# buttomnutstoast/Multigrid-Neural-Architectures

Hardware: NVIDIA B200
Metric: R-MG-34 train images/sec (higher is better)
Workload: dtype bf16

## Files before the change

### include/mgconv.h

```cpp
#ifndef MGCONV_H
#define MGCONV_H

#include <stdint.h>
#include <stddef.h>

#ifdef __cplusplus
extern "C" {
#endif

enum {
  MG_MAX_SEG = 6,
  MG_MAX_SRC = 8
};

typedef struct mg_ctx mg_ctx;

typedef enum {
  MG_OK = 0,
  MG_ERR_INVALID_ARG = 1,
  MG_ERR_SHAPE = 2,
  MG_ERR_CUDA = 3,
  MG_ERR_NCCL = 4,
  MG_ERR_UNSUPPORTED = 5
} mg_status;

typedef enum { MG_F32 = 0, MG_BF16 = 1 } mg_dtype;

typedef enum {
  MG_SEG_SAME = 0,
  MG_SEG_POOL = 1,
  MG_SEG_UP = 2
} mg_seg_mode;

typedef enum { MG_IMPL_AUTO = 0, MG_IMPL_SIMT = 1, MG_IMPL_TCGEN05 = 2 } mg_impl;

typedef struct { int64_t hi, lo; } mg_sum;

typedef struct {
  void* data;
  const float* scale;
  const float* shift;
  int32_t relu;
  int32_t N, H, W, C, Cp;
} mg_grid;

typedef struct {
  int32_t n_seg;
  mg_grid seg[MG_MAX_SEG];
  int32_t seg_mode[MG_MAX_SEG];
  int32_t ksize, stride, pad;
  int32_t Cout;
  int32_t H, W;
  int32_t algo_fwd, algo_bwd_data;
} mg_conv_desc;
enum { MG_ALGO_AUTO = 0, MG_ALGO_TILE128 = 1,
       MG_ALGO_TILE256 = 2,
       MG_ALGO_RESIDENT = 3,
       MG_ALGO_TILE128_DEEP = 4,
       MG_ALGO_TILE256_DEEP = 5,
       MG_ALGO_TILE128_MID = 6,
       MG_ALGO_PAIR128 = 7,
       MG_ALGO_PAIR256 = 8,
       MG_ALGO_RESIDENT_PAIR = 9 };

typedef struct {
  mg_grid g;
  int32_t c_offset;
  int32_t mode;
  const void* aux;
} mg_grad_src;

int mg_ctx_create(int device, void* cuda_stream, int dtype, mg_ctx** out);
int mg_ctx_destroy(mg_ctx* ctx);
int mg_ctx_set_stream(mg_ctx* ctx, void* cuda_stream);
int mg_ctx_set_impl(mg_ctx* ctx, int impl);
int mg_ctx_lane(mg_ctx* ctx, int lane);
int mg_ctx_event_record(mg_ctx* ctx, int ev);
int mg_ctx_event_wait(mg_ctx* ctx, int ev);
int mg_ctx_sync(mg_ctx* ctx);
enum { MG_TUNE_HALO_SUBTILES = 0,
       MG_TUNE_PERSISTENT = 1,
       MG_TUNE_STEM_FUSED_STATS = 2  };
int mg_ctx_set_tuning(mg_ctx* ctx, int knob, int value);
const char* mg_last_error(mg_ctx* ctx);
int mg_version(void);
int mg_ctx_launch_count(mg_ctx* ctx, int64_t* out);
int mg_ctx_tc_launch_count(mg_ctx* ctx, int64_t* out);
int mg_ctx_profile(mg_ctx* ctx, int on);
int mg_ctx_profile_read(mg_ctx* ctx, double* conv_ms, int64_t* conv_calls);

int mg_import_nchw(mg_ctx* ctx, const float* src, mg_grid* dst);
int mg_export_nchw(mg_ctx* ctx, const mg_grid* src, float* dst);

int mg_crop_flip_normalize(mg_ctx* ctx, const float* src, int32_t N, int32_t C, int32_t H, int32_t W, float* dst, int32_t oH, int32_t oW,
                           const int32_t* y0, const int32_t* x0, const int32_t* flip, const float* mean, const float* stdv);

size_t mg_conv_packed_bytes(const mg_conv_desc* d, int transposed);
int mg_conv_pack_weights(mg_ctx* ctx, const mg_conv_desc* d, const float* w, void* wpack, int transposed);
int mg_conv_pack_weights_batched(mg_ctx* ctx, int32_t n, const mg_conv_desc* const* descs, const float* const* w,
                                 void* const* wpack, const int32_t* transposed);

int mg_conv_forward(mg_ctx* ctx, const mg_conv_desc* d, const float* w, const void* wpack,
                    const float* bias, mg_grid* y, mg_sum* bn_sums);

int mg_bn_finalize(mg_ctx* ctx, const mg_sum* bn_sums, int64_t count, int32_t C, int32_t Cp,
                   const float* gamma, const float* beta, float* running_mean, float* running_var,
                   float eps, float momentum, int training,
                   float* scale, float* shift, float* save_mean, float* save_invstd);

int mg_residual_forward(mg_ctx* ctx, const mg_grid* z, const mg_grid* s, int relu, mg_grid* out, mg_grid* pooled);

typedef struct {
  const mg_sum* sums;
  int64_t count;
  const float* gamma;
  const float* beta;
// ... 89 lines not shown
```

### multigrid-neural-architectures_b200/csrc/umma_conv.cu

```cuda
#include "common.cuh"
#include "conv_view.cuh"
#include "umma_common.cuh"
#include "tma.cuh"
#include <algorithm>
#include <vector>

namespace {

constexpr int BM = 128;
constexpr int KV_PER_STAGE = 8;
constexpr int A_STAGE_BYTES = BM * 128;
constexpr int N_PRODUCERS = 128;
constexpr int MMA_WARP = 4, B_WARP = 5;
constexpr int N_THREADS = 192;
constexpr int MAX_STAGES = 8;

struct UParams {
  USeg seg[MG_MAX_SEG];
  int n_seg;
  int k, stride, pad;
  int H, W;
  int Ho, Wo;
  int64_t M;
  int Nimg;
// ... 267 lines not shown
    }
  }
  __syncthreads();
  if (warp == MMA_WARP) {
    tc_fence_after();
    asm volatile("tcgen05.dealloc.cta_group::1.sync.aligned.b32 %0, %1;" ::"r"(tmem_base), "r"(p.tmem_cols) : "memory");
  }
}



__device__ __forceinline__ float warp_reduce_scatter16(float (&v)[16], int lane) {
#pragma unroll
  for (int o = 8; o >= 1; o >>= 1) {
    const bool hi = (lane & o) != 0;
#pragma unroll
    for (int i = 0; i < o; ++i) {
      const float send = hi ? v[i] : v[i + o];
      const float keep = hi ? v[i + o] : v[i];
      v[i] = keep + __shfl_xor_sync(0xffffffffu, send, o);
    }
  }
  return v[0] + __shfl_xor_sync(0xffffffffu, v[0], 16);
}

constexpr int MAX_CHUNKS = 32;
struct HChunk { int seg, c0, nch, tps, ksteps, stage0; };

struct HParams {
  CUtensorMap tmap[MG_MAX_SEG];
  int seg_up[MG_MAX_SEG];
  HChunk chunk[MAX_CHUNKS];
  int n_seg, n_chunks, n_stages, any_up;
  int img_box;
  int H, W, Wp, Hp, Nimg;
  int64_t T;
  int HL;
  int nr_max;
  int halo_bytes;
  int n_abuf;
  int n_tile;
  const uint8_t* wpack;
  const float* bias;
  int c_bias;
  __nv_bfloat16* y;
  int y_pitch, c_valid;
  int stages, tmem_cols;
  mg_sum* stats;
  int c_stats;
  int m_tiles;
  CUtensorMap tmap_w;
  int tile_rows;
  int epi_stage;
};

__device__ __forceinline__ void zero_pad_column(uint8_t* a_smem, int nbuf, int halo_bytes, int nr_max, int Wp, int tid, int nthreads, int org = 0) {
  for (int i = tid; i < nbuf * nr_max * 8; i += nthreads) {
    const int q = i & 7, row = (i >> 3) % nr_max, buf = (i >> 3) / nr_max;
    *reinterpret_cast<uint4*>(a_smem + (size_t)buf * halo_bytes + (size_t)(org + row * Wp + Wp - 1) * 128 + q * 16) = make_uint4(0, 0, 0, 0);
  }
  fence_proxy_async();
}

__device__ __forceinline__ void zero_halo_margins(uint8_t* a_smem, int nbuf, int halo_bytes, int HL, int Wp, int tid, int nthreads) {
  const int m = Wp + 1;
  for (int i = tid; i < nbuf * 2 * m * 8; i += nthreads) {
    const int q = i & 7, sl = (i >> 3) % (2 * m), buf = (i >> 3) / (2 * m);
    const int slot = sl < m ? sl : HL - 2 * m + sl;
    *reinterpret_cast<uint4*>(a_smem + (size_t)buf * halo_bytes + (size_t)slot * 128 + q * 16) = make_uint4(0, 0, 0, 0);
  }
  fence_proxy_async();
}

__device__ __forceinline__ bool slot_pixel(const HParams& p, int64_t t, uint32_t* pix) {
  if (t >= p.T) return false;
  const uint32_t tu = (uint32_t)t, spi = (uint32_t)(p.Hp * p.Wp);
  const uint32_t n = tu / spi, rem = tu - n * spi;
  const uint32_t yy = rem / (uint32_t)p.Wp, xs = rem - yy * (uint32_t)p.Wp;
  if ((int)yy >= p.H || (int)xs >= p.W) return false;
  *pix = (n * p.H + yy) * p.W + xs;
  return true;
}

template <int MT>
__global__ void __launch_bounds__(32 * (4 * MT + 3), MT == 1 ? 4 : 2) umma_conv_halo_kernel(const __grid_constant__ HParams p) {
  constexpr int EPI_WARPS = 4 * MT, A_WARP = EPI_WARPS, B_WARP = EPI_WARPS + 1, M_WARP = EPI_WARPS + 2, NT = 32 * (EPI_WARPS + 3);
  extern __shared__ __align__(1024) uint8_t smem_raw[];
  uint8_t* smem = (uint8_t*)(((uintptr_t)smem_raw + 1023) & ~(uintptr_t)1023);
  __shared__ uint64_t full_bar[MAX_STAGES], empty_bar[MAX_STAGES], a_full[2], a_empty[2], tmem_full_bar;
  __shared__ uint32_t tmem_base_s;
  __shared__ float s_bias[256];

  pdl_launch();
  const int tid = threadIdx.x, warp = tid >> 5, lane = tid & 31;
  const int S = p.stages;
  const int b_stage_bytes = p.n_tile * 128;
  uint8_t* a_smem = smem;
  uint8_t* b_smem = smem + (size_t)p.n_abuf * p.halo_bytes;
  const int t0 = (int)blockIdx.x * (BM * MT);
  const int ntile = blockIdx.y;
  const int hs = t0 - p.Wp - 1;
  const int r0 = floordiv(hs, p.Wp);
  const int nr = (hs + p.HL - 1) / p.Wp - r0 + 1;
  const int off = p.img_box ? 0 : hs - r0 * p.Wp;

  if (tid == 0) {
// ... 735 lines not shown
          tma_load_rows_pair(&p.tmap[ch.seg], up, dst, &a_full[buf], ch.c0, r0, nr, p.W, p.Hp, lane);
        }
      }
    }
  } else if (warp == P_B_WARP) {
    if (lane == 0) {
      if (rank == 0) mbar_arrive_expect_tx(&b_full, (uint32_t)(2 * p.n_stages * b_half_bytes));
      for (int q = 0; q < p.n_stages; ++q)
        tma_load_2d_pair(smem_u32(b_smem + (size_t)q * b_half_bytes), &p.tmap_w, &b_full, 0, q * p.n_tile + (int)rank * (p.n_tile >> 1));
    }
  } else if (rank == 0) {
    const bool leader = elect_one();
    const uint32_t idesc = (1u << 4) | (1u << 7) | (1u << 10) | ((uint32_t)(p.n_tile >> 3) << 17) | ((uint32_t)(256 >> 4) << 24);
    const uint32_t b_base = smem_u32(b_smem);
    Ring ra(NA);
    mbar_wait_cluster(&b_full, 0);
    for (int it = 0; it < n_my; ++it) {
      const int acc = it & 1;
      if (it >= 2) { mbar_wait_cluster(&tmem_empty[acc], ((it >> 1) - 1) & 1); tc_fence_after(); }
      const uint32_t d_tmem = tmem_base + (uint32_t)(acc * p.n_tile);
      for (int c = 0; c < p.n_chunks; ++c, ra.next()) {
        const int buf = ra.idx;
        const HChunk ch = p.chunk[c];
        mbar_wait_cluster(&a_full[buf], ra.phase);
        tc_fence_after();
        const uint32_t a_base = smem_u32(a_smem + (size_t)buf * p.halo_bytes);
        const int tps = ch.tps, ksteps = ch.ksteps;
        const uint32_t sub_lo = 8u / (uint32_t)tps;
        if (leader) {
          int sub = 0, st = ch.stage0;
          for (int tap = 0; tap < 9; ++tap) {
            const uint32_t a_lo = desc_lo_k_sw128(a_base + (uint32_t)((tap / 3) * p.Wp + (tap % 3)) * 128u);
            const uint32_t b_lo = desc_lo_k_sw128(b_base + (uint32_t)(st * b_half_bytes)) + (uint32_t)sub * sub_lo;
#pragma unroll
            for (int q = 0; q < 4; ++q)
              if (q < ksteps) tc_mma_bf16_lohi_pair(d_tmem, a_lo + (uint32_t)(q * 2), b_lo + (uint32_t)(q * 2), DESC_HI_SW128, idesc, (uint32_t)((c | tap | q) != 0));
            if (++sub == tps) { sub = 0; ++st; }
          }
          tc_commit_pair(&a_empty[buf]);
        }
      }
      if (leader) tc_commit_pair(&tmem_full[acc]);
    }
  }
  __syncthreads();
  cluster_sync_all();
  if (warp == P_MMA_WARP) {
    tc_fence_after();
    asm volatile("tcgen05.dealloc.cta_group::2.sync.aligned.b32 %0, %1;" ::"r"(tmem_base), "r"(p.tmem_cols) : "memory");
  }
}


constexpr int ST_PC = 11, ST_PR = 37;
constexpr int ST_ROW = ST_PC * 16;
constexpr int ST_PLANE = 6592;
constexpr int ST_SLOT = 13312;
constexpr int ST_MAX_RING = 6;
constexpr int ST_RAW_COLS = 21;
constexpr int ST_RAW = 12544;
constexpr int ST_THREADS = 480;

struct StemParams {
  CUtensorMap tmap;
  CUtensorMap tmap_y;
  int tma_out;
  int H, W, Ho, Wo, Nimg;
  int tiles_x, tiles_y, n_tiles_total;
  int n_tile;
  int ring;
  const uint8_t* wpack;
  const float* bias; int c_bias;
  __nv_bfloat16* y; int y_pitch, c_valid;
  mg_sum* stats; int c_stats;
  int tmem_cols;
};

__device__ __forceinline__ uint64_t smem_desc_k_none(uint32_t saddr, uint32_t lbo_bytes, uint32_t sbo_bytes) {
  return (uint64_t)((saddr >> 4) & 0x3FFF) | ((uint64_t)((lbo_bytes >> 4) & 0x3FFF) << 16) | ((uint64_t)((sbo_bytes >> 4) & 0x3FFF) << 32) | (1ull << 46);
}

__global__ void __launch_bounds__(ST_THREADS, 1) umma_stem_kernel(const __grid_constant__ StemParams p) {
  pdl_launch();
  extern __shared__ __align__(1024) uint8_t smem_raw[];
  uint8_t* smem = (uint8_t*)(((uintptr_t)smem_raw + 1023) & ~(uintptr_t)1023);
  __shared__ uint64_t b_full, r_full[ST_MAX_RING], r_empty[ST_MAX_RING], a_full[ST_MAX_RING], a_empty[ST_MAX_RING], tmem_full[2], tmem_empty[2];
  __shared__ uint32_t tmem_base_s;

  const int tid = threadIdx.x, warp = tid >> 5, lane = tid & 31;
  const int NA = p.ring;
  const int b_stage_bytes = p.n_tile * 128;
  uint8_t* b_smem = smem;
  uint8_t* a_smem = smem + 7 * b_stage_bytes;
  uint8_t* r_smem = a_smem + (size_t)NA * ST_SLOT;
  uint8_t* o_smem = r_smem + (size_t)NA * ST_RAW;
  long long* s_part = reinterpret_cast<long long*>(o_smem + (p.tma_out ? 2 * 16384 : 0));
  float* s_bias = reinterpret_cast<float*>(s_part + 32 * p.n_tile);
  const int n_my = (p.n_tiles_total - (int)blockIdx.x + (int)gridDim.x - 1) / (int)gridDim.x;

  for (int c = tid; c < 32 * p.n_tile; c += ST_THREADS) s_part[c] = 0;
  if (tid == 0) {
    mbar_init(&b_full, 1);
    for (int s = 0; s < NA; ++s) { mbar_init(&a_full[s], 128); mbar_init(&a_empty[s], 1); mbar_init(&r_full[s], 1); mbar_init(&r_empty[s], 128); }
    for (int s = 0; s < 2; ++s) { mbar_init(&tmem_full[s], 1); mbar_init(&tmem_empty[s], 128); }
    asm volatile("fence.mbarrier_init.release.cluster;" ::: "memory");
  }
// ... 373 lines not shown
  if (!attr_set) {
    MG_CUDA(ctx, cudaFuncSetAttribute(umma_conv_kernel<true>, cudaFuncAttributeMaxDynamicSharedMemorySize, 227 * 1024 - 8 * 1024));
    MG_CUDA(ctx, cudaFuncSetAttribute(umma_conv_kernel<false>, cudaFuncAttributeMaxDynamicSharedMemorySize, 227 * 1024 - 8 * 1024));
    attr_set = true;
  }
  dim3 grid((unsigned)mg_cdiv(p.M, BM), (unsigned)n_tiles);
  bool fast = p.stride == 1 && (p.k == 1 || p.k == 3) && p.pad == p.k / 2 && p.Ho == p.H && p.Wo == p.W && p.M < (int64_t)1 << 31;
  for (int s = 0; s < p.n_seg; ++s) {
    if (p.seg[s].shift) fast = fast && p.seg[s].Hs == p.H / 2 && p.seg[s].Ws == p.W / 2 && p.H % 2 == 0 && p.W % 2 == 0;
    else fast = fast && p.seg[s].Hs == p.H && p.seg[s].Ws == p.W;
  }
  if (fast) umma_conv_kernel<true><<<grid, N_THREADS, smem, ctx->stream>>>(p);
  else umma_conv_kernel<false><<<grid, N_THREADS, smem, ctx->stream>>>(p);
  MG_CHECK_LAUNCH(ctx);
  ctx->tc_launches++;
  return MG_OK;
}

constexpr int SMEM_MAX = 232448 - 4096;

static void halo_geometry(HParams& p, int slots) {
  p.HL = slots + 2 * p.Wp + 2;
  p.nr_max = (p.HL - 1 + p.Wp - 1) / p.Wp + 1;
  p.halo_bytes = mg_round_up((p.img_box ? p.HL : p.nr_max * p.Wp) * 128, 1024);
}

static bool img_box_ok(const HParams& p, int slots) {
  static int on = -1;
  if (on < 0) { const char* e = getenv("MGCONV_IMG_BOX"); on = e ? atoi(e) : 1; }
  const int spi = p.Hp * p.Wp;
  return on && !p.any_up && slots % spi == 0 && slots / spi <= 256;
}

static int halo_tensor_maps(mg_ctx* ctx, HParams& p, const mg_grid* segs, int slots) {
  p.img_box = img_box_ok(p, slots) ? 1 : 0;
  for (int s = 0; s < p.n_seg; ++s) {
    const mg_grid& g = segs[s];
    int rc = p.img_box ? mg_tensor_map(ctx, g.data, p.Nimg, g.H, g.W, g.Cp, 4, slots / (p.Hp * p.Wp), &p.tmap[s])
                       : mg_tensor_map(ctx, g.data, p.Nimg, g.H, g.W, g.Cp, p.seg_up[s] ? 1 : 0, p.seg_up[s] ? 2 * g.W : p.Wp, &p.tmap[s]);
    if (rc) return rc;
  }
  return MG_OK;
}

static int epilogue_staging(const HParams& p, int MT, int smem_usable) {
  static int on = -1;
  if (on < 0) { const char* e = getenv("MGCONV_EPI_STAGE"); on = e ? atoi(e) : 1; }
  if (!on) return 0;
  const int off = p.stats ? MT * 4 * 2 * 256 * 4 : 0;
  const int need = off + MT * BM * (p.n_tile * 2 + 16);
  return need <= smem_usable ? off + 1 : 0;
}

static int launch_halo(mg_ctx* ctx, HParams& p, const Geometry& g, int algo, const mg_grid* segs) {
  const int b_stage = p.n_tile * 128;
  static int budget_env = -1, mt_env = -1;
  if (budget_env < 0) { const char* e = getenv("MGCONV_HALO_SMEM_KB"); budget_env = e ? atoi(e) : 0; }
  if (mt_env < 0) { const char* e = getenv("MGCONV_MT"); mt_env = e ? atoi(e) : 0; }
  int MT;
  {
    const int64_t ctas2 = mg_cdiv(p.T, 2 * BM) * g.n_tiles;
    const int want = (algo == MG_ALGO_TILE128 || algo == MG_ALGO_TILE128_DEEP || algo == MG_ALGO_TILE128_MID) ? 1
                     : ((algo == MG_ALGO_TILE256 || algo == MG_ALGO_TILE256_DEEP) ? 2 : (ctx->tune_mt ? ctx->tune_mt : mt_env));
    const bool heur2 = g.n_chunks >= 3 && ctas2 * 10 >= (int64_t)ctx->num_sms * 8;
    MT = (want == 1 || want == 2) ? want : (heur2 ? 2 : 1);
  }
  const bool pair = algo == MG_ALGO_PAIR128 || algo == MG_ALGO_PAIR256;
  if (pair) MT = algo == MG_ALGO_PAIR256 ? 2 : 1;
  { int rc = halo_tensor_maps(ctx, p, segs, BM * MT); if (rc) return rc; }
  halo_geometry(p, BM * MT);
  int cols = 32;
  while (cols < MT * p.n_tile) cols <<= 1;
  p.tmem_cols = cols;
  if (pair) {
    if (!p.img_box) p.halo_bytes = mg_round_up((p.nr_max * p.Wp + p.Wp) * 128, 1024);
    const int half = b_stage / 2;
    const int ctas = std::max(1, std::min(512 / cols, 2));
    int budget = (budget_env > 0 ? budget_env : (ctas == 1 ? 200 : 108)) * 1024;
    p.n_abuf = (g.n_chunks > 1 && 2 * p.halo_bytes + 2 * half <= budget) ? 2 : 1;
    int S = (budget - p.n_abuf * p.halo_bytes) / half;
    S = std::max(2, std::min(S, std::min(MAX_STAGES, p.n_stages)));
    p.stages = S;
    const int smem = p.n_abuf * p.halo_bytes + S * half + 1024;
    MG_REQUIRE(ctx, smem <= SMEM_MAX, MG_ERR_UNSUPPORTED, "pair halo conv: %d bytes of shared memory", smem);
    p.epi_stage = epilogue_staging(p, MT, smem - 1024);
    int rc = mg_tensor_map(ctx, p.wpack, g.n_tiles * p.n_stages * p.n_tile, 0, 0, 0, 5, p.n_tile / 2, &p.tmap_w);
    if (rc) return rc;
    static bool pair_attr_set = false;
    if (!pair_attr_set) {
      MG_CUDA(ctx, cudaFuncSetAttribute(umma_conv_halo_pair_kernel<1>, cudaFuncAttributeMaxDynamicSharedMemorySize, SMEM_MAX));
      MG_CUDA(ctx, cudaFuncSetAttribute(umma_conv_halo_pair_kernel<2>, cudaFuncAttributeMaxDynamicSharedMemorySize, SMEM_MAX));
      pair_attr_set = true;
    }
    dim3 grid((unsigned)mg_round_up((int)mg_cdiv(p.T, BM * MT), 2), (unsigned)g.n_tiles);
    if (MT == 2) MG_CUDA(ctx, mg_launch_pdl(umma_conv_halo_pair_kernel<2>, grid, dim3(32 * 11), (size_t)smem, ctx->stream, p));
    else MG_CUDA(ctx, mg_launch_pdl(umma_conv_halo_pair_kernel<1>, grid, dim3(32 * 7), (size_t)smem, ctx->stream, p));
    MG_CHECK_LAUNCH(ctx);
    ctx->tc_launches++;
    return MG_OK;
  }
  int budget_kb;
  if (MT == 1) {
    budget_kb = p.n_tile >= 192 ? 108 : 56;
  } else {
    const int ctas = std::max(1, std::min(512 / cols, 2));
    budget_kb = ctas == 1 ? 200 : 108;
  }
  if (algo == MG_ALGO_TILE128_MID) budget_kb = 72;
  if ((algo == MG_ALGO_AUTO || algo == MG_ALGO_RESIDENT) && mg_cdiv(p.T, BM * MT) * g.n_tiles <= ctx->num_sms) budget_kb = 200;
  if (algo == MG_ALGO_TILE128_DEEP) budget_kb = 108;
  if (algo == MG_ALGO_TILE256_DEEP) budget_kb = 200;
  if (budget_env > 0) budget_kb = budget_env;
  const int min_ring = 2;
  p.n_abuf = (g.n_chunks > 1 && 2 * p.halo_bytes + min_ring * b_stage <= budget_kb * 1024) ? 2 : 1;
  int S = (budget_kb * 1024 - p.n_abuf * p.halo_bytes) / b_stage;
  S = std::max(2, std::min(S, std::min(MAX_STAGES, p.n_stages)));
  p.stages = S;
  static bool attr_set = false;
  if (!attr_set) {
    MG_CUDA(ctx, cudaFuncSetAttribute(umma_conv_halo_kernel<1>, cudaFuncAttributeMaxDynamicSharedMemorySize, SMEM_MAX));
    MG_CUDA(ctx, cudaFuncSetAttribute(umma_conv_halo_kernel<2>, cudaFuncAttributeMaxDynamicSharedMemorySize, SMEM_MAX));
    attr_set = true;
  }
  const int smem = p.n_abuf * p.halo_bytes + S * b_stage + 1024;
  MG_REQUIRE(ctx, smem <= SMEM_MAX, MG_ERR_UNSUPPORTED, "halo conv: %d bytes of shared memory", smem);
  p.epi_stage = epilogue_staging(p, MT, smem - 1024);
  dim3 grid((unsigned)mg_cdiv(p.T, BM * MT), (unsigned)g.n_tiles);
  if (MT == 2) MG_CUDA(ctx, mg_launch_pdl(umma_conv_halo_kernel<2>, grid, dim3(32 * 11), (size_t)smem, ctx->stream, p));
  else MG_CUDA(ctx, mg_launch_pdl(umma_conv_halo_kernel<1>, grid, dim3(32 * 7), (size_t)smem, ctx->stream, p));
  MG_CHECK_LAUNCH(ctx);
  ctx->tc_launches++;
  return MG_OK;
}

struct PersistPlan { int n_abuf, smem, tmem_cols, grid, tile_rows, halo_bytes, pair; };
static int persist_tile_rows(const mg_conv_desc* d, int Nimg, bool any_up) {
  const int Wp = d->W + 1, Hp = d->H + 1;
  if (Wp > BM) return 0;
  if (!any_up && BM % (Hp * Wp) == 0) return 0;
  const int R = BM / Wp;
  if (R < 1 || R * Wp * 100 < BM * 85) return 0;
  (void)Nimg;
  return R;
}
static bool persist_plan(const mg_ctx* ctx, const mg_conv_desc* d, const Geometry& g, int Nimg, int algo, bool stats, PersistPlan* pl) {
  static int on = -1, min_tiles_per_sm = -1;
  if (on < 0) { const char* e = getenv("MGCONV_PERSIST"); on = e ? atoi(e) : 1; }
  if (min_tiles_per_sm < 0) { const char* e = getenv("MGCONV_PERSIST_MIN_TILES"); min_tiles_per_sm = e ? atoi(e) : 4; }
  if (algo == MG_ALGO_TILE128 || algo == MG_ALGO_TILE256 || algo == MG_ALGO_TILE128_DEEP || algo == MG_ALGO_TILE256_DEEP ||
      algo == MG_ALGO_TILE128_MID || algo == MG_ALGO_PAIR128 || algo == MG_ALGO_PAIR256) return false;
  const bool pair = algo == MG_ALGO_RESIDENT_PAIR;
  const bool forced = algo == MG_ALGO_RESIDENT || pair || ctx->tune_persist == 1;
  if (!forced && (ctx->tune_persist == 2 || !on)) return false;
  if (!g.halo || g.n_tiles != 1) return false;
  HParams hp;
  hp.Wp = d->W + 1; hp.img_box = 0;
  halo_geometry(hp, BM);
  bool any_up = false;
  for (int s = 0; s < d->n_seg; ++s) any_up = any_up || d->seg_mode[s] == MG_SEG_UP;
  static int aligned_single = -1;
  if (aligned_single < 0) { const char* e = getenv("MGCONV_PERSIST_ALIGNED"); aligned_single = e ? atoi(e) : 0; }
  const int R = ((pair || aligned_single) && !stats) ? persist_tile_rows(d, Nimg, any_up && g.n_chunks > 0) : 0;
  if (R) hp.halo_bytes = mg_round_up(((R + 2) * hp.Wp + 2) * 128, 1024);
  const int64_t m_tiles = R ? mg_cdiv((int64_t)Nimg * (d->H + 1), R) : mg_cdiv((int64_t)Nimg * (d->H + 1) * hp.Wp, BM);
  if (!forced && m_tiles < (int64_t)min_tiles_per_sm * ctx->num_sms) return false;
  if (pair && !R && !(!any_up && BM % ((d->H + 1) * hp.Wp) == 0)) return false;
  const int b_bytes = g.n_stages * g.n_tile * (pair ? 64 : 128);
  const int tail = g.n_tile * (4 + 256);
  const int room = SMEM_MAX - 1024 - b_bytes - tail;
  int n_abuf = room / hp.halo_bytes;
  if (n_abuf < 2) return false;
  n_abuf = std::min(n_abuf, std::min(P_MAX_ABUF, 2 * g.n_chunks + 1));
  int cols = 32;
  while (cols < 2 * g.n_tile) cols <<= 1;
  if (cols > 512) return false;
  pl->n_abuf = n_abuf; pl->smem = n_abuf * hp.halo_bytes + b_bytes + tail + 1024; pl->tmem_cols = cols;
  pl->grid = (int)std::min<int64_t>(m_tiles, ctx->num_sms);
  if (pair) pl->grid = 2 * (int)std::min<int64_t>((m_tiles + 1) / 2, ctx->num_sms / 2);
  pl->tile_rows = R; pl->halo_bytes = hp.halo_bytes; pl->pair = pair ? 1 : 0;
  return true;
}

static int launch_halo_persistent(mg_ctx* ctx, HParams& p, const PersistPlan& pl, const mg_grid* segs) {
  { int rc = halo_tensor_maps(ctx, p, segs, BM); if (rc) return rc; }
  halo_geometry(p, BM);
  p.m_tiles = (int)mg_cdiv(p.T, BM);
  p.tile_rows = p.img_box ? 0 : pl.tile_rows;
  if (p.tile_rows) {
    p.halo_bytes = pl.halo_bytes;
    p.nr_max = p.tile_rows + 2;
    p.m_tiles = (int)mg_cdiv((int64_t)p.Nimg * p.Hp, p.tile_rows);
  }
  p.tmem_cols = pl.tmem_cols;
  p.n_abuf = pl.n_abuf;
  p.stages = 0;
  static bool attr_set = false;
  if (!attr_set) {
    MG_CUDA(ctx, cudaFuncSetAttribute(umma_conv_halo_persistent_kernel, cudaFuncAttributeMaxDynamicSharedMemorySize, SMEM_MAX));
    attr_set = true;
  }
  if (pl.pair) {
    int rc = mg_tensor_map(ctx, p.wpack, p.n_stages * p.n_tile, 0, 0, 0, 5, p.n_tile / 2, &p.tmap_w);
    if (rc) return rc;
// ... 239 lines not shown
```

### multigrid-neural-architectures_b200/mgconv/engine.py

```python
import ctypes as C
import os
import torch

from . import ffi, lower, ops, sched

_PRECISION = {"bf16": (ffi.MG_BF16, torch.bfloat16), "fp32": (ffi.MG_F32, torch.float32)}
_IMPL = {"auto": ffi.MG_IMPL_AUTO, "simt": ffi.MG_IMPL_SIMT, "tcgen05": ffi.MG_IMPL_TCGEN05}
_crit_ctx = {}


def criterion_ctx(t):
    if not t.is_cuda:
        raise ffi.MGError("criterion inputs must be CUDA tensors: the multigrid hot path has no CPU fallback")
    dev = t.device.index
    if dev not in _crit_ctx:
        _crit_ctx[dev] = ffi.Context(dev, 0, ffi.MG_F32)
    _crit_ctx[dev].set_stream(torch.cuda.current_stream(dev).cuda_stream)
    return _crit_ctx[dev]


def _flatten(x):
    if isinstance(x, (list, tuple)):
        out = []
        for e in x:
# ... 41 lines not shown
                if w.device != self.device:
                    raise ffi.MGError(f"{m.typename} parameters live on {w.device}, inputs on {self.device}: call model:cuda()")

        shapes = [tuple(t.shape) for t in inputs]
        b, out = lower.trace_model(model, shapes if isinstance(input, (list, tuple)) else shapes[0],
                                   bool(getattr(model, "needInputGrad", False)))
        self.out_struct = self._wrap_outputs(out, b)
        self.plan = b
        self.input_ops = [o for o in b.ops if isinstance(o, ops.InputOp)]
        self.conv_ops = [o for o in b.ops if isinstance(o, ops.ConvOp)]
        ops.fuse_stem_pool3(b.ops, self)
        for o in b.ops:
            o.setup_fwd(self)
        self._bwd_ready = False

    def _wrap_outputs(self, out, b):
        if isinstance(out, (list, tuple)):
            return [self._wrap_outputs(e, b) for e in out]
        if isinstance(out, lower.OutVal):
            return out.op
        if isinstance(out, lower.CatVal):
            out = b.as_tensor(out)
        if isinstance(out, lower.TVal):
            return b.emit(ops.ExportOp(out.spec))
        raise NotImplementedError(f"model output of kind {type(out).__name__}")

    def alloc(self, shape, dtype=None):
        t = torch.zeros(shape, dtype=dtype or self.elt, device=self.device)
        self.bytes += t.numel() * t.element_size()
        return t

    def alloc_sums(self, n, which):
        arena = self._sums[which]
        n2 = 2 * n
        n8 = (n2 + 7) // 8 * 8
        if arena[1] + n8 > arena[0].numel():
            raise ffi.MGError("BatchNorm statistics arena exhausted")
        v = arena[0][arena[1]:arena[1] + n2]
        arena[1] += n8
        return v

    def zero_sums(self, which):
        arena = self._sums[which]
        if arena[1]:
            self.ctx.call("mg_memset_zero", ffi.ptr(arena[0]), arena[1] * 8)

    def param_done(self, mod):
        if self.on_param_done is not None:
            self.on_param_done(mod)

    def _report_tuning(self, field):
        if os.environ.get("MGCONV_VERBOSE"):
            import collections
            names = {0: "heuristic", 1: "tile128", 2: "tile256", 3: "resident", 4: "tile128deep", 5: "tile256deep", 6: "tile128mid"}
            cnt = collections.Counter((o.H, o.CcatP, o.Cout, names[getattr(o.desc, field)]) for o in self.conv_ops if o._tunable())
            print(f"[mgconv] autotune {field}: " + ", ".join(f"{h}x{h} {ci}->{co}: {a} x{n}" for (h, ci, co, a), n in sorted(cnt.items())), flush=True)

    def set_bn_sync(self, nranks):
        self.bn_sync = int(nranks)

    def _use_lanes(self):
        return self.n_lanes > 1 and not self.bn_sync

    def invalidate_schedules(self):
        self._sched_fwd = self._sched_bwd = None

    def _bind_stream(self):
        self.ctx.set_stream(torch.cuda.current_stream(self.device).cuda_stream)

    def pack_weights(self):
        import ctypes as C
        jobs = [j for o in self.conv_ops for j in o.pack_jobs()]
        if not jobs:
            return
        key = tuple((id(d), w.data_ptr(), wp.data_ptr(), t) for d, w, wp, t in jobs)
        if self._pack_cache is None or self._pack_cache[0] != key:
            n = len(jobs)
            descs = (C.POINTER(ffi.mg_conv_desc) * n)(*[C.pointer(d) for d, _, _, _ in jobs])
            ws = (C.c_void_p * n)(*[w.data_ptr() for _, w, _, _ in jobs])
            wps = (C.c_void_p * n)(*[wp.data_ptr() for _, _, wp, _ in jobs])
            tr = (C.c_int32 * n)(*[t for _, _, _, t in jobs])
            self._pack_cache = (key, n, descs, ws, wps, tr)
        _, n, descs, ws, wps, tr = self._pack_cache
        self.ctx.call("mg_conv_pack_weights_batched", n, descs, ws, wps, tr)

    def forward(self, input, training=True):
        self._bind_stream()
        self.training = training
        for op, t in zip(self.input_ops, _flatten(input)):
            op.src = t.contiguous().float()
        self.pack_weights()
        if self.autotune and not self._tuned_fwd and self.use_packed and not torch.cuda.is_current_stream_capturing():
            self._tuned_fwd = True
            for o in self.conv_ops:
                o.tune_fwd(self)
            self._report_tuning("algo_fwd")
        self.zero_sums("fwd")
        if self._use_lanes():
            if self._sched_fwd is None:
                self._sched_fwd = sched.Schedule(self.plan.ops, lambda o: o.io_fwd(), lambda o: o.fwd, self.n_lanes, 0)
            self._sched_fwd.run(self)
        elif self.bn_sync and training:
            self._run_sync_bn(self.plan.ops, fwd=True)
        else:
            for o in self.plan.ops:
                o.fwd(self)
        return self._results(self.out_struct)
# ... 82 lines not shown
```

### multigrid-neural-architectures_b200/mgconv/ffi.py

```python
import ctypes as C
import os

MG_MAX_SEG = 6
MG_MAX_SRC = 8
MG_F32, MG_BF16 = 0, 1
MG_SEG_SAME, MG_SEG_POOL, MG_SEG_UP, MG_SRC_POOL3 = 0, 1, 2, 3
MG_IMPL_AUTO, MG_IMPL_SIMT, MG_IMPL_TCGEN05 = 0, 1, 2
MG_TUNE_HALO_SUBTILES, MG_TUNE_PERSISTENT, MG_TUNE_STEM_FUSED_STATS = 0, 1, 2
MG_ALGO_AUTO, MG_ALGO_TILE128, MG_ALGO_TILE256, MG_ALGO_RESIDENT, MG_ALGO_TILE128_DEEP, MG_ALGO_TILE256_DEEP, MG_ALGO_TILE128_MID = 0, 1, 2, 3, 4, 5, 6
MG_ALGO_PAIR128, MG_ALGO_PAIR256, MG_ALGO_RESIDENT_PAIR = 7, 8, 9

_HERE = os.path.dirname(os.path.abspath(__file__))
LIB_PATH = os.environ.get("MGCONV_LIB", os.path.join(_HERE, "libmgconv.so"))


class MGError(RuntimeError):
    pass


class mg_grid(C.Structure):
    _fields_ = [("data", C.c_void_p), ("scale", C.c_void_p), ("shift", C.c_void_p), ("relu", C.c_int32),
                ("N", C.c_int32), ("H", C.c_int32), ("W", C.c_int32), ("C", C.c_int32), ("Cp", C.c_int32)]


class mg_conv_desc(C.Structure):
    _fields_ = [("n_seg", C.c_int32), ("seg", mg_grid * MG_MAX_SEG), ("seg_mode", C.c_int32 * MG_MAX_SEG),
                ("ksize", C.c_int32), ("stride", C.c_int32), ("pad", C.c_int32), ("Cout", C.c_int32),
                ("H", C.c_int32), ("W", C.c_int32), ("algo_fwd", C.c_int32), ("algo_bwd_data", C.c_int32)]


class mg_grad_src(C.Structure):
    _fields_ = [("g", mg_grid), ("c_offset", C.c_int32), ("mode", C.c_int32), ("aux", C.c_void_p)]


MG_STAGE_MAX_GRIDS = 4


class mg_stage_desc(C.Structure):
    _fields_ = [("n_scales", C.c_int32), ("C_in", C.c_int32 * MG_STAGE_MAX_GRIDS), ("C_out", C.c_int32 * MG_STAGE_MAX_GRIDS),
                ("H", C.c_int32 * MG_STAGE_MAX_GRIDS), ("W", C.c_int32 * MG_STAGE_MAX_GRIDS), ("ksize", C.c_int32 * MG_STAGE_MAX_GRIDS),
                ("residual", C.c_int32), ("no_final_relu", C.c_int32), ("eps", C.c_float), ("momentum", C.c_float)]


class mg_stage_params(C.Structure):
    _fields_ = [(name, C.c_void_p * (2 * MG_STAGE_MAX_GRIDS)) for name in
                ("conv_w", "conv_b", "bn_g", "bn_b", "bn_rm", "bn_rv", "conv_gw", "conv_gb", "bn_gg", "bn_gb")]


class mg_bn_fused(C.Structure):
    _fields_ = [("sums", C.c_void_p), ("count", C.c_int64), ("gamma", C.c_void_p), ("beta", C.c_void_p),
                ("running_mean", C.c_void_p), ("running_var", C.c_void_p), ("eps", C.c_float), ("momentum", C.c_float),
                ("training", C.c_int32), ("save_mean", C.c_void_p), ("save_invstd", C.c_void_p)]


def _load():
    if not os.path.exists(LIB_PATH):
        raise MGError(
            f"{LIB_PATH} not found: build it with `make -C multigrid-neural-architectures_b200/csrc` "
            "(or __graft_entry__.build()); there is no CPU / PyTorch fallback for the multigrid hot path")
    return C.CDLL(LIB_PATH, mode=C.RTLD_GLOBAL)


lib = _load()
# ... 135 lines not shown
```

### multigrid-neural-architectures_b200/mgconv/ops.py

```python
import ctypes as C
import os
import torch

from . import ffi
from .ffi import mg_grid, mg_conv_desc, mg_grad_src, mg_bn_fused, ptr, MG_SEG_SAME, MG_SEG_POOL, MG_SEG_UP, MG_SRC_POOL3, MG_MAX_SRC


def cpad(c):
    return (c + 7) // 8 * 8


def _k(x):
    if x is None:
        return None
    if isinstance(x, torch.Tensor):
        return x.data_ptr()
    if isinstance(x, mg_grid):
        return x.data
    return int(x)


def _keys(*xs):
    return [k for k in (_k(x) for x in xs) if k]

# ... 176 lines not shown
        d = mg_conv_desc()
        d.n_seg = len(self.segs)
        for i, (t, m) in enumerate(self.segs):
            d.seg[i] = t.grid()
            d.seg_mode[i] = m
        d.ksize, d.stride, d.pad, d.Cout, d.H, d.W = self.k, self.stride, self.pad, self.Cout, self.H, self.W
        self.desc = d
        self.y.buf = E.alloc(self.y.shape())
        self.yg = self.y.grid()
        if self.want_stats:
            self.sums = E.alloc_sums(2 * self.Cout, "fwd")
        t0 = self.segs[0][0]
        self.col = None
        if (E.use_packed and len(self.segs) == 1 and self.segs[0][1] == MG_SEG_SAME and self.stride > 1 and self.k > 1
                and t0.C * self.k * self.k <= 512 and not t0.needs_grad and os.environ.get("MGCONV_STEM_IM2COL", "0") == "1"):
            K = t0.C * self.k * self.k
            Kp = cpad(K)
            self.col = E.alloc((self.y.N, self.Ho, self.Wo, Kp))
            self.col_g = mg_grid(self.col.data_ptr(), None, None, 0, self.y.N, self.Ho, self.Wo, K, Kp)
            self.in_g = t0.grid()
            d1 = mg_conv_desc()
            d1.n_seg = 1
            d1.seg[0] = self.col_g
            d1.seg_mode[0] = MG_SEG_SAME
            d1.ksize, d1.stride, d1.pad, d1.Cout, d1.H, d1.W = 1, 1, 0, self.Cout, self.Ho, self.Wo
            self.desc_direct, self.desc = d, d1
        self.wpack = self.wpack_t = None
        nb = ffi.lib.mg_conv_packed_bytes(C.byref(self.desc), 0) if E.use_packed else 0
        if nb:
            self.wpack = E.alloc((nb,), torch.uint8)
        self.Ccat = sum(t.C for t, _ in self.segs)
        self.CcatP = sum(t.Cp for t, _ in self.segs)

    def pack(self, E):
        if self.wpack is not None:
            E.ctx.call("mg_conv_pack_weights", C.byref(self.desc), ptr(self.mod.weight), ptr(self.wpack), 0)
        if self.wpack_t is not None:
            E.ctx.call("mg_conv_pack_weights", C.byref(self.desc), ptr(self.mod.weight), ptr(self.wpack_t), 1)

    def pack_jobs(self):
        jobs = []
        if self.wpack is not None:
            jobs.append((self.desc, self.mod.weight, self.wpack, 0))
        if self.wpack_t is not None:
            jobs.append((self.desc, self.mod.weight, self.wpack_t, 1))
        return jobs

    def _tunable(self):
        return self.wpack is not None and self.k == 3 and self.stride == 1 and self.pad == 1 and 7 <= self.W <= 63

    def _pick(self, E, field, run):
        best, best_t = 0, None
        for algo in (ffi.MG_ALGO_TILE128, ffi.MG_ALGO_TILE256, ffi.MG_ALGO_RESIDENT, ffi.MG_ALGO_TILE128_DEEP, ffi.MG_ALGO_TILE256_DEEP,
                     ffi.MG_ALGO_TILE128_MID, ffi.MG_ALGO_PAIR128, ffi.MG_ALGO_PAIR256, ffi.MG_ALGO_RESIDENT_PAIR):
            setattr(self.desc, field, algo)
            run()
            e0, e1 = torch.cuda.Event(enable_timing=True), torch.cuda.Event(enable_timing=True)
            e0.record()
            for _ in range(3):
                run()
            e1.record()
            e1.synchronize()
            t = e0.elapsed_time(e1)
            if best_t is None or t < best_t * 0.97:
                best, best_t = algo, t
        setattr(self.desc, field, best)
        return best

    def tune_fwd(self, E):
        if self._tunable():
            self._pick(E, "algo_fwd", lambda: self.fwd(E))

    def tune_bwd(self, E):
        if self._tunable() and self.needs_dgrad and self.wpack_t is not None:
            g = self.y.G
            self._pick(E, "algo_bwd_data", lambda: E.ctx.call("mg_conv_backward_data", C.byref(self.desc), ptr(self.mod.weight),
                                                              ptr(self.wpack_t), C.byref(g), C.byref(self.dcat_g)))

    def size(self):
        return self.H

    def io_fwd(self):
        return _keys(*[t.buf for t, _ in self.segs]), _keys(self.y.buf, self.sums, self.col)

    def io_bwd(self):
        io = self.ycomb.io() if self.ycomb is not None else None
        r = _keys(self.y.G, self.col, *[t.buf for t, _ in self.segs])
        w = _keys(self.mod.gradWeight, self.mod.gradBias, self.dcat)
        return _merge(io, (r, w))

    def fwd(self, E):
        if self.col is not None:
            E.ctx.call("mg_im2col", C.byref(self.in_g), self.k, self.stride, self.pad, C.byref(self.col_g))
        E.ctx.call("mg_conv_forward", C.byref(self.desc), ptr(self.mod.weight), ptr(self.wpack), ptr(self.mod.bias),
                   C.byref(self.yg), ptr(self.sums))

    def setup_bwd(self, E):
        if self.apply is None:
            self.ycomb = Combine(E, self.y)
            self.y.G = self.ycomb.grid()
        self.needs_dgrad = any(t.needs_grad for t, _ in self.segs)
        self.dcat = None
        if self.needs_dgrad:
            self.dcat = E.alloc((self.y.N, self.H, self.W, self.CcatP))
            self.dcat_g = mg_grid(self.dcat.data_ptr(), None, None, 0, self.y.N, self.H, self.W, self.CcatP, self.CcatP)
            off = 0
            for t, m in self.segs:
# ... 460 lines not shown
```

Measured before the change: 15260.

## Add stream-pair conv algo with tail-balanced N-slicing for autotuner

Adds a new cluster-pair tcgen05 halo conv kernel that walks a static list of (M-tile pair, N-tile) units across SM pairs. It splits the leftover tail units into column slices of a tuned width so the final wave is spread evenly over all pairs. The aim is to cut wave-quantization idle time on the last round. It is offered to the per-layer autotuner as one more candidate, so it only runs where it measures faster, at the cost of extra tuning time and a second weight tensor map.

```diff
diff --git a/include/mgconv.h b/include/mgconv.h
--- a/include/mgconv.h
+++ b/include/mgconv.h
@@ -61,7 +61,8 @@
        MG_ALGO_TILE128_MID = 6,
        MG_ALGO_PAIR128 = 7,
        MG_ALGO_PAIR256 = 8,
-       MG_ALGO_RESIDENT_PAIR = 9 };
+       MG_ALGO_RESIDENT_PAIR = 9,
+       MG_ALGO_STREAM_PAIR = 10 };
 
 typedef struct {
   mg_grid g;
diff --git a/multigrid-neural-architectures_b200/csrc/umma_conv.cu b/multigrid-neural-architectures_b200/csrc/umma_conv.cu
--- a/multigrid-neural-architectures_b200/csrc/umma_conv.cu
+++ b/multigrid-neural-architectures_b200/csrc/umma_conv.cu
@@ -343,6 +343,9 @@
   CUtensorMap tmap_w;
   int tile_rows;
   int epi_stage;
+  int n_ntiles;
+  int s_units, s_pairs, s_rounds, s_q;
+  CUtensorMap tmap_wt;
 };
 
 __device__ __forceinline__ void zero_pad_column(uint8_t* a_smem, int nbuf, int halo_bytes, int nr_max, int Wp, int tid, int nthreads, int org = 0) {
@@ -1184,6 +1187,247 @@
 }
 
 
+struct SUnit { int pt, nt, c0, ns; };
+
+__device__ __forceinline__ int stream_tail_cols(const HParams& p) { return (p.s_units - p.s_rounds * p.s_pairs) * p.n_tile; }
+
+__device__ __forceinline__ int stream_units(const HParams& p, int pair) {
+  const int tail = stream_tail_cols(p), l0 = pair * p.s_q;
+  if (l0 >= tail) return p.s_rounds;
+  const int l1 = min(l0 + p.s_q, tail) - 1;
+  return p.s_rounds + l1 / p.n_tile - l0 / p.n_tile + 1;
+}
+
+__device__ __forceinline__ SUnit stream_unit(const HParams& p, int pair, int i) {
+  int u, c0 = 0, ns = p.n_tile;
+  if (i < p.s_rounds) {
+    u = pair + i * p.s_pairs;
+  } else {
+    const int l0 = pair * p.s_q, l1 = min(l0 + p.s_q, stream_tail_cols(p));
+    const int l = i == p.s_rounds ? l0 : (l0 / p.n_tile + 1) * p.n_tile;
+    const int k = l / p.n_tile;
+    c0 = l - k * p.n_tile;
+    ns = min(l1, (k + 1) * p.n_tile) - l;
+    u = p.s_rounds * p.s_pairs + k;
+  }
+  return SUnit{u / p.n_ntiles, u % p.n_ntiles, c0, ns};
+}
+
+__global__ void __cluster_dims__(2, 1, 1) __launch_bounds__(P_THREADS, 1) umma_conv_halo_stream_pair_kernel(const __grid_constant__ HParams p) {
+  pdl_launch();
+  extern __shared__ __align__(1024) uint8_t smem_raw[];
+  uint8_t* smem = (uint8_t*)(((uintptr_t)smem_raw + 1023) & ~(uintptr_t)1023);
+  __shared__ uint64_t full_bar[MAX_STAGES], empty_bar[MAX_STAGES], a_full[P_MAX_ABUF], a_empty[P_MAX_ABUF], tmem_full[2], tmem_empty[2];
+  __shared__ uint32_t tmem_base_s;
+  __shared__ float s_bias[512];
+
+  const int tid = threadIdx.x, warp = tid >> 5, lane = tid & 31;
+  const uint32_t rank = cluster_ctarank();
+  const int NA = p.n_abuf, S = p.stages;
+  const int b_half_bytes = (p.n_tile >> 1) * 128;
+  uint8_t* a_smem = smem;
+  uint8_t* b_smem = smem + (size_t)NA * p.halo_bytes;
+  float* s_part = reinterpret_cast<float*>(b_smem + (size_t)S * b_half_bytes);
+  const int pair = (int)blockIdx.x >> 1;
+  const int n_my = stream_units(p, pair);
+  const int a_first = p.img_box ? 0 : p.Wp;
+
+  if (tid == 0) {
+    for (int s = 0; s < S; ++s) { mbar_init(&full_bar[s], 1); mbar_init(&empty_bar[s], 1); }
+    for (int s = 0; s < NA; ++s) { mbar_init(&a_full[s], 2); mbar_init(&a_empty[s], 1); }
+    for (int s = 0; s < 2; ++s) { mbar_init(&tmem_full[s], 1); mbar_init(&tmem_empty[s], 256); }
+    asm volatile("fence.mbarrier_init.release.cluster;" ::: "memory");
+  }
+  if (warp == P_MMA_WARP) {
+    asm volatile("tcgen05.alloc.cta_group::2.sync.aligned.shared::cta.b32 [%0], %1;" ::"r"(smem_u32(&tmem_base_s)), "r"(p.tmem_cols) : "memory");
+    asm volatile("tcgen05.relinquish_alloc_permit.cta_group::2.sync.aligned;" ::: "memory");
+  }
+  if (warp == P_A_WARP && lane < p.n_seg) tma_prefetch_desc(&p.tmap[lane]);
+  if (warp == P_B_WARP && lane == 0) { tma_prefetch_desc(&p.tmap_w); tma_prefetch_desc(&p.tmap_wt); }
+  if (p.img_box) zero_halo_margins(a_smem, NA, p.halo_bytes, p.HL, p.Wp, tid, P_THREADS);
+  pdl_wait();
+  for (int c = tid; c < p.n_ntiles * p.n_tile; c += P_THREADS) s_bias[c] = (p.bias && c < p.c_bias) ? p.bias[c] : 0.f;
+  tc_fence_before();
+  __syncthreads();
+  cluster_sync_all();
+  tc_fence_after();
+  const uint32_t tmem_base = tmem_base_s;
+
+  if (warp < 8) {
+    const int grp = warp >> 2, qw = warp & 3, row = qw * 32 + lane;
+    const bool want_stats = p.stats != nullptr;
+    float* sp = s_part + grp * (4 * 2 * 256);
+    for (int it = grp; it < n_my; it += 2) {
+      const SUnit u = stream_unit(p, pair, it);
+      const int acc = it & 1;
+      uint32_t pix = 0;
+      const bool row_ok = slot_pixel(p, (int64_t)(2 * u.pt + (int)rank) * BM + row, &pix);
+      const int nb = u.nt * p.n_tile + u.c0;
+      mbar_wait_cluster(&tmem_full[acc], (it >> 1) & 1);
+      tc_fence_after();
+      __nv_bfloat16* yrow = p.y + (size_t)pix * p.y_pitch;
+      const uint32_t tcol = tmem_base + ((uint32_t)(qw * 32) << 16) + (uint32_t)(acc * p.n_tile);
+      for (int c0 = 0; c0 < u.ns; c0 += 16) {
+        uint32_t a16[16];
+        tc_ld16(tcol + (uint32_t)c0, a16);
+        tc_wait_ld();
+        uint32_t pk[2][4];
+#pragma unroll
+        for (int h = 0; h < 2; ++h) {
+          const int n0 = nb + c0 + h * 8;
+#pragma unroll
+          for (int e = 0; e < 4; ++e) {
+            const float a = __uint_as_float(a16[h * 8 + 2 * e]) + s_bias[n0 + 2 * e];
+            const float b = __uint_as_float(a16[h * 8 + 2 * e + 1]) + s_bias[n0 + 2 * e + 1];
+            __nv_bfloat162 t2 = __floats2bfloat162_rn(a, b);
+            pk[h][e] = *reinterpret_cast<uint32_t*>(&t2);
+          }
+          if (row_ok && n0 + 8 <= p.c_valid) *reinterpret_cast<uint4*>(yrow + n0) = make_uint4(pk[h][0], pk[h][1], pk[h][2], pk[h][3]);
+        }
+        if (want_stats) {
+#pragma unroll
+          for (int h = 0; h < 2; ++h) {
+            const bool use = row_ok && nb + c0 + h * 8 + 8 <= p.c_valid;
+            float sv[16];
+#pragma unroll
+            for (int e = 0; e < 4; ++e) {
+              const float ra = use ? __uint_as_float(pk[h][e] << 16) : 0.f, rb = use ? __uint_as_float(pk[h][e] & 0xFFFF0000u) : 0.f;
+              sv[2 * e] = ra; sv[2 * e + 1] = rb;
+              sv[8 + 2 * e] = ra * ra; sv[8 + 2 * e + 1] = rb * rb;
+            }
+            const float tot = warp_reduce_scatter16(sv, lane);
+            if (lane < 16) sp[(qw * 2 + (lane >> 3)) * 256 + c0 + h * 8 + (lane & 7)] = tot;
+          }
+        }
+      }
+      tc_fence_before();
+      mbar_arrive_cluster(&tmem_empty[acc], 0);
+      if (want_stats) {
+        asm volatile("bar.sync %0, 128;" ::"r"(1 + grp) : "memory");
+        for (int c = row; c < u.ns; c += 128) {
+          const int ch = nb + c;
+          if (ch < p.c_stats) {
+            long long ah = 0, al = 0, bh = 0, bl = 0, h, l;
+#pragma unroll
+            for (int w = 0; w < 4; ++w) {
+              mg_to_fix_f32(sp[(2 * w) * 256 + c], h, l); ah += h; al += l;
+              mg_to_fix_f32(sp[(2 * w + 1) * 256 + c], h, l); bh += h; bl += l;
+            }
+            mg_sum_add_fix(p.stats + ch, ah, al);
+            mg_sum_add_fix(p.stats + p.c_stats + ch, bh, bl);
+          }
+        }
+        asm volatile("bar.sync %0, 128;" ::"r"(1 + grp) : "memory");
+      }
+    }
+  } else if (warp == P_A_WARP) {
+    Ring ra(NA);
+    int ac = 0;
+    for (int it = 0; it < n_my; ++it) {
+      const SUnit u = stream_unit(p, pair, it);
+      const int t0 = (2 * u.pt + (int)rank) * BM;
+      const int hs = t0 - p.Wp - 1;
+      const int r0 = floordiv(hs, p.Wp);
+      const int nr = (hs + p.HL - 1) / p.Wp - r0 + 1;
+      const int org = p.Wp - (hs - r0 * p.Wp);
+      const int hs_p = 2 * u.pt * BM + BM - p.Wp - 1;
+      const int r0_p = floordiv(hs_p, p.Wp);
+      const int nr_p = (hs_p + p.HL - 1) / p.Wp - r0_p + 1;
+      for (int c = 0; c < p.n_chunks; ++c, ++ac, ra.next()) {
+        const int buf = ra.idx;
+        if (ac >= NA) mbar_wait_cluster(&a_empty[buf], ra.phase ^ 1u);
+        const HChunk ch = p.chunk[c];
+        uint8_t* abuf = a_smem + (size_t)buf * p.halo_bytes;
+        const uint32_t dst = smem_u32(abuf);
+        if (p.img_box) {
+          if (lane == 0) {
+            if (rank == 0) mbar_arrive_expect_tx(&a_full[buf], 2u * (uint32_t)BM * 128u);
+            tma_load_4d_pair(dst + (uint32_t)(p.Wp + 1) * 128u, &p.tmap[ch.seg], &a_full[buf], ch.c0, 0, 0, t0 / (p.Hp * p.Wp));
+          }
+        } else {
+          const int up = p.seg_up[ch.seg];
+          if (up) {
+            for (int i = lane; i < nr * 8; i += 32)
+              *reinterpret_cast<uint4*>(abuf + (size_t)(org + (i >> 3) * p.Wp + p.Wp - 1) * 128 + (i & 7) * 16) = make_uint4(0, 0, 0, 0);
+            fence_proxy_async();
+          }
+          __syncwarp();
+          if (rank == 0 && lane == 0) mbar_arrive_expect_tx(&a_full[buf], (uint32_t)(nr + nr_p) * (uint32_t)(up ? p.W : p.Wp) * 128u);
+          __syncwarp();
+          tma_load_rows_pair(&p.tmap[ch.seg], up, dst + (uint32_t)org * 128u, &a_full[buf], ch.c0, r0, nr, p.W, p.Hp, lane);
+        }
+        if (rank == 1 && lane == 0) mbar_arrive_cluster(&a_full[buf], 0);
+      }
+    }
+  } else if (warp == P_B_WARP) {
+    if (lane == 0) {
+      Ring rb(S);
+      int ks_all = 0;
+      for (int it = 0; it < n_my; ++it) {
+        const SUnit u = stream_unit(p, pair, it);
+        const bool whole = u.ns == p.n_tile;
+        const CUtensorMap* tm = whole ? &p.tmap_w : &p.tmap_wt;
+        const uint32_t bytes = (uint32_t)(whole ? p.n_tile : p.s_q) * 128u;
+        const int row0 = u.nt * p.n_stages * p.n_tile + u.c0 + (int)rank * (u.ns >> 1);
+        for (int ks = 0; ks < p.n_stages; ++ks, ++ks_all, rb.next()) {
+          const int s = rb.idx;
+          if (ks_all >= S) mbar_wait_cluster(&empty_bar[s], rb.phase ^ 1u);
+          if (rank == 0) mbar_arrive_expect_tx(&full_bar[s], bytes);
+          tma_load_2d_pair(smem_u32(b_smem + (size_t)s * b_half_bytes), tm, &full_bar[s], 0, row0 + ks * p.n_tile);
+        }
+      }
+    }
+  } else if (rank == 0) {
+    const bool leader = elect_one();
+    Ring ra(NA), rb(S);
+    for (int it = 0; it < n_my; ++it) {
+      const SUnit u = stream_unit(p, pair, it);
+      const int acc = it & 1;
+      const uint32_t idesc = (1u << 4) | (1u << 7) | (1u << 10) | ((uint32_t)(u.ns >> 3) << 17) | ((uint32_t)(256 >> 4) << 24);
+      if (it >= 2) { mbar_wait_cluster(&tmem_empty[acc], ((it >> 1) - 1) & 1); tc_fence_after(); }
+      const uint32_t d_tmem = tmem_base + (uint32_t)(acc * p.n_tile);
+      for (int c = 0; c < p.n_chunks; ++c, ra.next()) {
+        const int buf = ra.idx;
+        const HChunk ch = p.chunk[c];
+        mbar_wait_cluster(&a_full[buf], ra.phase);
+        tc_fence_after();
+        const uint32_t a_base = smem_u32(a_smem + (size_t)buf * p.halo_bytes) + (uint32_t)a_first * 128u;
+        const int tps = ch.tps, ksteps = ch.ksteps;
+        const uint32_t sub_lo = 8u / (uint32_t)tps;
+        int sub = 0;
+        uint32_t b_lo = 0;
+        for (int tap = 0; tap < 9; ++tap) {
+          if (sub == 0) {
+            mbar_wait_cluster(&full_bar[rb.idx], rb.phase);
+            tc_fence_after();
+            b_lo = desc_lo_k_sw128(smem_u32(b_smem + (size_t)rb.idx * b_half_bytes));
+          }
+          const uint32_t a_lo = desc_lo_k_sw128(a_base + (uint32_t)((tap / 3) * p.Wp + (tap % 3)) * 128u);
+          const bool last_of_stage = (sub == tps - 1) || tap == 8;
+          if (leader) {
+#pragma unroll
+            for (int q = 0; q < 4; ++q)
+              if (q < ksteps)
+                tc_mma_bf16_lohi_pair(d_tmem, a_lo + (uint32_t)(q * 2), b_lo + (uint32_t)sub * sub_lo + (uint32_t)(q * 2), DESC_HI_SW128, idesc,
+                                      (uint32_t)((c | tap | q) != 0));
+            if (last_of_stage) tc_commit_pair(&empty_bar[rb.idx]);
+          }
+          if (last_of_stage) { sub = 0; rb.next(); } else ++sub;
+        }
+        if (leader) tc_commit_pair(&a_empty[buf]);
+      }
+      if (leader) tc_commit_pair(&tmem_full[acc]);
+    }
+  }
+  __syncthreads();
+  cluster_sync_all();
+  if (warp == P_MMA_WARP) {
+    tc_fence_after();
+    asm volatile("tcgen05.dealloc.cta_group::2.sync.aligned.b32 %0, %1;" ::"r"(tmem_base), "r"(p.tmem_cols) : "memory");
+  }
+}
+
+
 constexpr int ST_PC = 11, ST_PR = 37;
 constexpr int ST_ROW = ST_PC * 16;
 constexpr int ST_PLANE = 6592;
@@ -1663,7 +1907,77 @@
   return need <= smem_usable ? off + 1 : 0;
 }
 
+static int stream_tail_q(const HParams& p, const Geometry& g, int tail_cols, int P) {
+  int kmma = 0;
+  for (int c = 0; c < g.n_chunks; ++c) kmma += 9 * g.chunk[c].ksteps;
+  const double halo = (double)g.n_chunks * (p.img_box ? BM : p.nr_max * p.Wp) * 128;
+  auto slice = [&](int ns, int q) {
+    const double mma = kmma * std::max(44.0, 137.0 * ns / 256.0);
+    return std::max(mma, (halo + (double)g.n_stages * (q / 2) * 128) / 40.0);
+  };
+  int best_q = p.n_tile;
+  double best = -1;
+  for (int q = mg_round_up(mg_cdiv(tail_cols, P), 16); q <= p.n_tile; q += 16) {
+    double worst = 0;
+    for (int l0 = 0; l0 < tail_cols; l0 += q) {
+      const int l1 = std::min(l0 + q, tail_cols), cut = (l0 / p.n_tile + 1) * p.n_tile;
+      worst = std::max(worst, l1 <= cut ? slice(l1 - l0, q) : slice(cut - l0, q) + slice(l1 - cut, q));
+    }
+    if (best < 0 || worst < best) { best = worst; best_q = q; }
+  }
+  return best_q;
+}
+
+static bool stream_pair_plan(HParams& p, const Geometry& g, int* smem) {
+  if (g.n_tiles * p.n_tile > 512) return false;
+  p.img_box = img_box_ok(p, BM) ? 1 : 0;
+  halo_geometry(p, BM);
+  if (!p.img_box) p.halo_bytes = mg_round_up((p.nr_max * p.Wp + p.Wp) * 128, 1024);
+  int cols = 32;
+  while (cols < 2 * p.n_tile) cols <<= 1;
+  p.tmem_cols = cols;
+  const int half = p.n_tile * 64;
+  const int stats_bytes = p.stats ? 2 * 4 * 2 * 256 * 4 : 0;
+  const int room = SMEM_MAX - 1024 - stats_bytes;
+  p.n_abuf = std::min(3, std::max(2, g.n_chunks + 1));
+  if ((room - p.n_abuf * p.halo_bytes) / half < 4) p.n_abuf = 2;
+  p.stages = std::min(MAX_STAGES, (room - p.n_abuf * p.halo_bytes) / half);
+  if (p.stages < 2) return false;
+  *smem = p.n_abuf * p.halo_bytes + p.stages * half + stats_bytes + 1024;
+  return true;
+}
+
+static int launch_halo_stream_pair(mg_ctx* ctx, HParams& p, const Geometry& g, const mg_grid* segs, int smem) {
+  { int rc = halo_tensor_maps(ctx, p, segs, BM); if (rc) return rc; }
+  p.m_tiles = (int)mg_cdiv(p.T, BM);
+  p.n_ntiles = g.n_tiles;
+  p.s_units = (p.m_tiles + 1) / 2 * g.n_tiles;
+  p.s_pairs = std::max(1, ctx->num_sms / 2);
+  p.s_rounds = p.s_units / p.s_pairs;
+  const int tail_cols = (p.s_units - p.s_rounds * p.s_pairs) * p.n_tile;
+  p.s_q = tail_cols ? stream_tail_q(p, g, tail_cols, p.s_pairs) : p.n_tile;
+  const int pairs = p.s_rounds ? p.s_pairs : (int)mg_cdiv(tail_cols, p.s_q);
+  const int rows = g.n_tiles * p.n_stages * p.n_tile;
+  int rc = mg_tensor_map(ctx, p.wpack, rows, 0, 0, 0, 5, p.n_tile / 2, &p.tmap_w);
+  if (!rc) rc = mg_tensor_map(ctx, p.wpack, rows, 0, 0, 0, 5, p.s_q / 2, &p.tmap_wt);
+  if (rc) return rc;
+  static bool attr_set = false;
+  if (!attr_set) {
+    MG_CUDA(ctx, cudaFuncSetAttribute(umma_conv_halo_stream_pair_kernel, cudaFuncAttributeMaxDynamicSharedMemorySize, SMEM_MAX));
+    attr_set = true;
+  }
+  MG_CUDA(ctx, mg_launch_pdl(umma_conv_halo_stream_pair_kernel, dim3(2 * pairs), dim3(P_THREADS), (size_t)smem, ctx->stream, p));
+  MG_CHECK_LAUNCH(ctx);
+  ctx->tc_launches++;
+  return MG_OK;
+}
+
 static int launch_halo(mg_ctx* ctx, HParams& p, const Geometry& g, int algo, const mg_grid* segs) {
+  if (algo == MG_ALGO_STREAM_PAIR) {
+    int smem = 0;
+    if (stream_pair_plan(p, g, &smem)) return launch_halo_stream_pair(ctx, p, g, segs, smem);
+    algo = MG_ALGO_AUTO;
+  }
   const int b_stage = p.n_tile * 128;
   static int budget_env = -1, mt_env = -1;
   if (budget_env < 0) { const char* e = getenv("MGCONV_HALO_SMEM_KB"); budget_env = e ? atoi(e) : 0; }
@@ -1759,7 +2073,7 @@
   if (on < 0) { const char* e = getenv("MGCONV_PERSIST"); on = e ? atoi(e) : 1; }
   if (min_tiles_per_sm < 0) { const char* e = getenv("MGCONV_PERSIST_MIN_TILES"); min_tiles_per_sm = e ? atoi(e) : 4; }
   if (algo == MG_ALGO_TILE128 || algo == MG_ALGO_TILE256 || algo == MG_ALGO_TILE128_DEEP || algo == MG_ALGO_TILE256_DEEP ||
-      algo == MG_ALGO_TILE128_MID || algo == MG_ALGO_PAIR128 || algo == MG_ALGO_PAIR256) return false;
+      algo == MG_ALGO_TILE128_MID || algo == MG_ALGO_PAIR128 || algo == MG_ALGO_PAIR256 || algo == MG_ALGO_STREAM_PAIR) return false;
   const bool pair = algo == MG_ALGO_RESIDENT_PAIR;
   const bool forced = algo == MG_ALGO_RESIDENT || pair || ctx->tune_persist == 1;
   if (!forced && (ctx->tune_persist == 2 || !on)) return false;
diff --git a/multigrid-neural-architectures_b200/mgconv/engine.py b/multigrid-neural-architectures_b200/mgconv/engine.py
--- a/multigrid-neural-architectures_b200/mgconv/engine.py
+++ b/multigrid-neural-architectures_b200/mgconv/engine.py
@@ -117,7 +117,8 @@
     def _report_tuning(self, field):
         if os.environ.get("MGCONV_VERBOSE"):
             import collections
-            names = {0: "heuristic", 1: "tile128", 2: "tile256", 3: "resident", 4: "tile128deep", 5: "tile256deep", 6: "tile128mid"}
+            names = {0: "heuristic", 1: "tile128", 2: "tile256", 3: "resident", 4: "tile128deep", 5: "tile256deep", 6: "tile128mid",
+                     7: "pair128", 8: "pair256", 9: "residentpair", 10: "streampair"}
             cnt = collections.Counter((o.H, o.CcatP, o.Cout, names[getattr(o.desc, field)]) for o in self.conv_ops if o._tunable())
             print(f"[mgconv] autotune {field}: " + ", ".join(f"{h}x{h} {ci}->{co}: {a} x{n}" for (h, ci, co, a), n in sorted(cnt.items())), flush=True)
 
diff --git a/multigrid-neural-architectures_b200/mgconv/ffi.py b/multigrid-neural-architectures_b200/mgconv/ffi.py
--- a/multigrid-neural-architectures_b200/mgconv/ffi.py
+++ b/multigrid-neural-architectures_b200/mgconv/ffi.py
@@ -8,7 +8,7 @@
 MG_IMPL_AUTO, MG_IMPL_SIMT, MG_IMPL_TCGEN05 = 0, 1, 2
 MG_TUNE_HALO_SUBTILES, MG_TUNE_PERSISTENT, MG_TUNE_STEM_FUSED_STATS = 0, 1, 2
 MG_ALGO_AUTO, MG_ALGO_TILE128, MG_ALGO_TILE256, MG_ALGO_RESIDENT, MG_ALGO_TILE128_DEEP, MG_ALGO_TILE256_DEEP, MG_ALGO_TILE128_MID = 0, 1, 2, 3, 4, 5, 6
-MG_ALGO_PAIR128, MG_ALGO_PAIR256, MG_ALGO_RESIDENT_PAIR = 7, 8, 9
+MG_ALGO_PAIR128, MG_ALGO_PAIR256, MG_ALGO_RESIDENT_PAIR, MG_ALGO_STREAM_PAIR = 7, 8, 9, 10
 
 _HERE = os.path.dirname(os.path.abspath(__file__))
 LIB_PATH = os.environ.get("MGCONV_LIB", os.path.join(_HERE, "libmgconv.so"))
diff --git a/multigrid-neural-architectures_b200/mgconv/ops.py b/multigrid-neural-architectures_b200/mgconv/ops.py
--- a/multigrid-neural-architectures_b200/mgconv/ops.py
+++ b/multigrid-neural-architectures_b200/mgconv/ops.py
@@ -252,7 +252,7 @@
     def _pick(self, E, field, run):
         best, best_t = 0, None
         for algo in (ffi.MG_ALGO_TILE128, ffi.MG_ALGO_TILE256, ffi.MG_ALGO_RESIDENT, ffi.MG_ALGO_TILE128_DEEP, ffi.MG_ALGO_TILE256_DEEP,
-                     ffi.MG_ALGO_TILE128_MID, ffi.MG_ALGO_PAIR128, ffi.MG_ALGO_PAIR256, ffi.MG_ALGO_RESIDENT_PAIR):
+                     ffi.MG_ALGO_TILE128_MID, ffi.MG_ALGO_PAIR128, ffi.MG_ALGO_PAIR256, ffi.MG_ALGO_RESIDENT_PAIR, ffi.MG_ALGO_STREAM_PAIR):
             setattr(self.desc, field, algo)
             run()
             e0, e1 = torch.cuda.Event(enable_timing=True), torch.cuda.Event(enable_timing=True)
```

New measurement: 15210 (median of 6 runs). No clear change (-0.3%).
